# ChunLI-666/PointCloudProcessor

Hardware: AMD Instinct MI355X
Metric: Mpoints×frames/sec colorized (higher is better)
Workload: dtype f32/f64

## Files before the change

### include/pcp_hip.h

```cpp
#ifndef PCP_HIP_H
#define PCP_HIP_H

#include <stdint.h>

#ifdef __cplusplus
extern "C" {
#endif

#define PCP_ABI_VERSION 6

#define PCP_OK 0
#define PCP_ERR_INVALID (-1)
#define PCP_ERR_STATE (-2)
#define PCP_ERR_DEVICE (-3)
#define PCP_ERR_NOMEM (-4)
#define PCP_ERR_RANGE (-5)

typedef struct pcp_context pcp_context;

typedef struct pcp_pose {
  double x, y, z, qw, qx, qy, qz;
} pcp_pose;

typedef struct pcp_camera {
// ... 191 lines not shown
                   int64_t capacity, char *out_text, int64_t *out_bytes);
int pcp_colour_compact_ascii(pcp_context *ctx, int32_t with_label, int64_t first_row, int64_t max_rows, int64_t capacity,
                             char *out_text, int64_t *out_rows, int64_t *out_bytes);
int pcp_mls_fetch_ascii(pcp_context *ctx, int64_t first_row, int64_t max_rows, int64_t capacity, char *out_text,
                        int64_t *out_rows, int64_t *out_bytes);

#define PCP_ASCII_PARSE_MAX_ROW 65536
#define PCP_PARSE_LIMIT_ROW 0
#define PCP_PARSE_LIMIT_TILE 1
#define PCP_PARSE_LIMIT_PIECE 2
#define PCP_PARSE_LIMIT_TILE_ROWS 3
#define PCP_PARSE_LIMIT_WINDOW 4
int64_t pcp_ascii_parse_limit(int32_t which);
int pcp_ascii_parse_host(const char *text, int64_t bytes, int32_t columns, const int32_t col[4], int32_t final_window,
                         int64_t max_rows, float *out_x, float *out_y, float *out_z, float *out_intensity,
                         int64_t *out_rows, int64_t *out_consumed, int64_t *out_bad_row);
int pcp_ascii_parse(pcp_context *ctx, const char *text, int64_t bytes, int32_t columns, const int32_t col[4], int32_t final_window,
                    int64_t max_rows, float *out_x, float *out_y, float *out_z, float *out_intensity,
                    int64_t *out_rows, int64_t *out_consumed, int64_t *out_bad_row);

int pcp_close_pairs(pcp_context *ctx, double radius, int64_t *points_with_close_neighbour);

int pcp_timing_enable(pcp_context *ctx, int32_t on);
int pcp_timing_reset(pcp_context *ctx);
int pcp_timing_get(pcp_context *ctx, int32_t kernel_id, double *total_ms, int64_t *launches);
const char *pcp_kernel_name(int32_t kernel_id);
int pcp_tile_mask_density(pcp_context *ctx, double *kept_fraction);
int pcp_tile_masks(pcp_context *ctx, int64_t *tiles, int32_t *mask_words, uint32_t *out_words);
int pcp_sor_redo_fraction(pcp_context *ctx, double *fraction);
int pcp_sor_distances(pcp_context *ctx, int64_t capacity, float *out_distance);
int pcp_selftest_arithmetic(pcp_context *ctx, int64_t samples, uint64_t seed, int64_t *mismatches_fp64,
                            int64_t *mismatches_fp32);

#ifdef __cplusplus
}
#endif
#endif
```

### pointcloudprocessor_amd/capi.py

```python
from __future__ import annotations

import ctypes as C
import os
import re

import numpy as np

from . import _build

PCP_OK = 0
PCP_ERR_INVALID = -1
PCP_ERR_STATE = -2
PCP_ERR_DEVICE = -3
PCP_ERR_NOMEM = -4
PCP_ERR_RANGE = -5

NID_EVAL_FN = C.CFUNCTYPE(C.c_int, C.c_void_p, C.POINTER(C.c_double), C.c_int32, C.POINTER(C.c_double), C.POINTER(C.c_double),
                          C.POINTER(C.c_int32))
K_PROJECT, K_DEPTH, K_COLOUR, K_VISIBILITY, K_MLS_GRID, K_MLS_FIT, K_MISC, K_SOR, K_MLS_VOXEL, K_TILE_MASK, K_NID, K_HPR = range(12)
K_COLOUR_SMOOTH = 12
K_COUNT = 13


class PcpError(RuntimeError):
# ... 755 lines not shown
        Ti = np.ascontiguousarray(T_init, np.float64).reshape(16)
        out = np.zeros(16, np.float64)
        cost = C.c_double()
        evals = C.c_int32()
        rc = self.lib.pcp_nid_optimize_with(self.h, trampoline, None, _ptr(Ti), C.c_int32(bins), C.c_int32(max_outer_iterations),
                                            _ptr(out), C.byref(cost), C.byref(evals))
        if errors:
            raise errors[0]
        self._check(rc)
        return out.reshape(4, 4), cost.value, evals.value

    def timing_enable(self, on: bool = True):
        self._check(self.lib.pcp_timing_enable(self.h, C.c_int32(1 if on else 0)))

    def timing_reset(self):
        self._check(self.lib.pcp_timing_reset(self.h))

    def timing_get(self, kernel_id: int):
        ms = C.c_double()
        cnt = C.c_int64()
        self._check(self.lib.pcp_timing_get(self.h, C.c_int32(kernel_id), C.byref(ms), C.byref(cnt)))
        return ms.value, cnt.value

    def tile_mask_density(self) -> float:
        v = C.c_double()
        self._check(self.lib.pcp_tile_mask_density(self.h, C.byref(v)))
        return v.value

    def selftest_arithmetic(self, samples: int = 1 << 26, seed: int = 1):
        a, b = C.c_int64(), C.c_int64()
        self._check(self.lib.pcp_selftest_arithmetic(self.h, C.c_int64(samples), C.c_uint64(seed), C.byref(a), C.byref(b)))
        return a.value, b.value

    def tile_masks(self) -> np.ndarray:
        t, w = C.c_int64(), C.c_int32()
        self._check(self.lib.pcp_tile_masks(self.h, C.byref(t), C.byref(w), None))
        out = np.empty((t.value, w.value), np.uint32)
        self._check(self.lib.pcp_tile_masks(self.h, None, None, _ptr(out)))
        return out

    def kernel_name(self, kernel_id: int) -> str:
        return self.lib.pcp_kernel_name(C.c_int32(kernel_id)).decode()
```

### pointcloudprocessor_amd/csrc/pcp_colour.hip

```cpp
#include <algorithm>
#include <cfloat>
#include <cstdlib>

#include "pcp_device.hpp"
#include "pcp_hsv.hpp"
#include "pcp_scan.hpp"

namespace pcp {

constexpr int kBlock = 256;
constexpr uint32_t kFltMaxBits = 0x7f7fffffu;

template <bool kCommon>
__device__ __forceinline__ DevCamera common_camera(const DevCamera &in) {
  DevCamera c = in;
  if constexpr (kCommon) {
    c.cull_mode = PCP_CULL_ZBUFFER;
    c.enable_zbuf = 1;
    c.pretest = 1;
    c.ds_fast = 1;
  }
  return c;
}
inline bool is_common_camera(const DevCamera &c) {
// ... 291 lines not shown
  const uint32_t b = blockIdx.x;
  if (b >= (gridDim.x / kSuper) * kSuper) return b;
  const uint32_t x = b % kXcd, slot = b / kXcd;
  return ((slot / kXcdChunk) * kXcd + x) * kXcdChunk + slot % kXcdChunk;
}

constexpr unsigned long long kDepthEmpty = 0x7f7f7f7f7f7f7f7full;
__device__ __forceinline__ void depth_min(unsigned long long *__restrict__ map, int32_t cell, unsigned long long bits) {
  if (bits < map[cell]) atomicMin(map + cell, bits);
}
__device__ __forceinline__ double sumsq64(float xc, float yc, float zc) {
  const double X = xc, Y = yc, Z = zc;
  return (X * X + Y * Y) + Z * Z;
}
__global__ __launch_bounds__(kBlock) void k_depth_finish(const unsigned long long *__restrict__ sq, int64_t count,
                                                         uint32_t *__restrict__ range) {
  int64_t i = static_cast<int64_t>(blockIdx.x) * kBlock + threadIdx.x;
  const int64_t stride = static_cast<int64_t>(gridDim.x) * kBlock;
  for (; i < count; i += stride) {
    const unsigned long long b = sq[i];
    float r = FLT_MAX;
    if (b != kDepthEmpty) r = fminf(static_cast<float>(sqrt(__longlong_as_double(static_cast<long long>(b)))), FLT_MAX);
    range[i] = __float_as_uint(r);
  }
}

__device__ __forceinline__ uint32_t range_bits(int32_t w, int32_t f0, int32_t f1) {
  const int32_t fb = max(f0, w << 5), fe = min(f1, (w << 5) + 32);
  const int32_t nb = fe - fb;
  return nb <= 0 ? 0u : (((nb >= 32) ? 0xffffffffu : ((1u << nb) - 1u)) << (fb & 31));
}

template <bool kCommon>
__global__ __launch_bounds__(kBlock) void k_depth_pass(const float *__restrict__ x, const float *__restrict__ y,
                                                       const float *__restrict__ z, int64_t n, DevCamera cam_in,
                                                       const DevFrame *__restrict__ frames, int32_t f0, int32_t f1,
                                                       unsigned long long *__restrict__ depth, int64_t cells,
                                                       int32_t depth_first_frame, uint32_t *__restrict__ tile_mask,
                                                       const uint32_t *__restrict__ tile_inside, int32_t words,
                                                       const int32_t *__restrict__ tile_order) {
  DevCamera cam = common_camera<kCommon>(cam_in);
  if constexpr (kCommon) cam.pretest = 0;
  __shared__ unsigned long long combine[kBlock];
  const int lane = threadIdx.x & 63;
  unsigned long long *tbl = combine + (threadIdx.x & ~63);
  const int64_t j = tile_order ? static_cast<int64_t>(tile_order[blockIdx.x]) * 64 + threadIdx.x
                               : static_cast<int64_t>(xcd_chunked_block()) * kBlock + threadIdx.x;
  const bool live = j < n;
  if (!__ballot(live)) return;
  const float px = live ? x[j] : 0.0f, py = live ? y[j] : 0.0f, pz = live ? z[j] : 0.0f;
  const int64_t tile = __builtin_amdgcn_readfirstlane(static_cast<int32_t>(j >> 6));
  const bool finite_sure = cam.frames_bounded != 0 && __all(fabsf(px) <= 0x1p40f && fabsf(py) <= 0x1p40f && fabsf(pz) <= 0x1p40f);
  unsigned long long *held_at = nullptr;
  unsigned long long held_bits = 0ull, held_seen = 0ull;
  auto settle_held = [&]() {
    if (held_at && held_bits < held_seen) atomicMin(held_at, held_bits);
    held_at = nullptr;
  };
  for (int32_t w = f0 >> 5; w <= (f1 - 1) >> 5; ++w) {
    const uint32_t in_range = range_bits(w, f0, f1);
    uint32_t todo = in_range;
    if (tile_mask) todo &= tile_mask[tile * words + w];
    todo = __builtin_amdgcn_readfirstlane(todo);
    const uint32_t inside = tile_inside ? __builtin_amdgcn_readfirstlane(tile_inside[tile * words + w]) : 0u;
    uint32_t seen = 0u;
    while (todo) {
      const int32_t b = __builtin_ctz(todo);
      const int32_t f = (w << 5) + b;
      todo &= todo - 1u;
      const DevFrame &fr = frames[f];
      const Projected p = project_point(cam, fr.w2c, px, py, pz, ((inside >> b) & 1u) == 0u, finite_sure);
      const bool in_map = live && p.cell >= 0;
      const bool cand = live && p.pixel >= 0 && (cam.enable_zbuf ? p.cell >= 0 : p.cell != -1);
      if (__ballot(cand)) seen |= 1u << b;
      settle_held();
      if (cam.enable_zbuf && __ballot(in_map)) {
        unsigned long long *map = depth + static_cast<uint64_t>(static_cast<uint32_t>(f - depth_first_frame)) * static_cast<uint32_t>(cells);
        unsigned long long key = ~0ull, sbits = 0ull;
        if (in_map) {
          sbits = static_cast<unsigned long long>(__double_as_longlong(sumsq64(p.xc, p.yc, p.zc)));
          key = (static_cast<unsigned long long>(static_cast<uint32_t>(p.cell)) << 32) | (sbits >> 32);
        }
        tbl[lane] = ~0ull;
        __builtin_amdgcn_wave_barrier();
        if (in_map) atomicMin(&tbl[p.cell & 63], key);
        __builtin_amdgcn_wave_barrier();
        if (in_map) {
          const unsigned long long got = tbl[p.cell & 63];
          if (got == key || static_cast<uint32_t>(got >> 32) != static_cast<uint32_t>(p.cell)) {
            held_at = map + p.cell;
            held_bits = sbits;
            held_seen = *held_at;
          }
        }
        __builtin_amdgcn_wave_barrier();
      }
    }
    if (tile_mask && lane == 0 && live) {
      uint32_t *dst = tile_mask + tile * words + w;
      *dst = (*dst & ~in_range) | seen;
    }
  }
  settle_held();
}

__global__ __launch_bounds__(kBlock) void k_visibility(const float *__restrict__ x, const float *__restrict__ y,
                                                       const float *__restrict__ z, int64_t n, DevCamera cam,
                                                       DevFrame fr, const uint32_t *__restrict__ depth,
                                                       const int32_t *__restrict__ perm,
                                                       uint8_t *__restrict__ keep, int32_t require_pixel) {
  const int64_t i = static_cast<int64_t>(blockIdx.x) * kBlock + threadIdx.x;
  if (i >= n) return;
  const Projected p = project_point(cam, fr.w2c, x[i], y[i], z[i]);
  bool k = keep_rule(cam, p, depth);
  if (require_pixel) k = k && p.pixel >= 0;
  if (k) keep[perm ? perm[i] : i] = 1;
}

__device__ __forceinline__ bool keep_by_depth(float xc, float yc, float zc, double lim) {
  const double s = sumsq64(xc, yc, zc);
  const double L = lim * lim;
  bool keep = s < L * (1.0 - 0x1p-40);
  const bool sure = lim > 0.0 && (keep || s > L * (1.0 + 0x1p-40));
  if (!sure) keep = !(sqrt(s) > lim);
  return keep;
}

struct TopState {
  float *score;
  uint32_t *rgb;
  int32_t *frame;
  int32_t *count;
};

struct MatchArgs {
  const uint8_t *in_a;
  unsigned long long *moved;
  float e2;
// ... 224 lines not shown
  const uint64_t a = mix64(seed ^ static_cast<uint64_t>(i) * 3u), b = mix64(a);
  uint32_t bx = static_cast<uint32_t>(a), by = static_cast<uint32_t>(a >> 32), bz = static_cast<uint32_t>(b);
  const uint32_t mode = static_cast<uint32_t>(b >> 32) & 3u;
  if (mode != 0u) {
    const uint32_t span = mode == 1u ? 12u : 40u;
    bx = (bx & 0x807fffffu) | ((127u - span / 2u + (bx >> 23) % span) << 23);
    by = (by & 0x807fffffu) | ((127u - span / 2u + (by >> 23) % span) << 23);
    bz = (bz & 0x807fffffu) | ((127u - span / 2u + (bz >> 23) % span) << 23);
  }
  const float xc = __uint_as_float(bx), yc = __uint_as_float(by), zc = fabsf(__uint_as_float(bz));
  if (!(zc > 0.0f)) return;
  double xn, yn;
  divide_xy_by_z(xc, yc, zc, xn, yn);
  const double xr = static_cast<double>(xc) / static_cast<double>(zc);
  const double yr = static_cast<double>(yc) / static_cast<double>(zc);
  if (!same_f64(xn, xr) || !same_f64(yn, yr)) atomicAdd(bad, 1ull);
}

__global__ __launch_bounds__(kBlock) void k_selftest_div32(DevCamera cam, unsigned long long *__restrict__ bad) {
  const uint32_t lane = blockIdx.x * kBlock + threadIdx.x;
  uint32_t wrong = 0u;
  for (uint32_t k = 0; k < 256u; ++k) {
    const float x = __uint_as_float((k << 24) | lane);
    const float a = div_by_ds(cam, x), b = x / cam.ds_f;
    const float ax = fabsf(x);
    if (ax >= 0x1p-40f && ax <= 0x1p60f) {
      if (!((a != a && b != b) || __float_as_uint(a) == __float_as_uint(b))) ++wrong;
    } else {
      if (cell_of_quotient(a, cam.cull_wf) != cell_of_quotient(b, cam.cull_wf)) ++wrong;
      if (cell_of_quotient(a, cam.cull_hf) != cell_of_quotient(b, cam.cull_hf)) ++wrong;
    }
  }
  if (wrong) atomicAdd(bad, static_cast<unsigned long long>(wrong));
}

__global__ __launch_bounds__(kBlock) void k_unpack_result(const uint32_t *__restrict__ packed, int64_t n,
                                                         uint8_t *__restrict__ rgb, uint8_t *__restrict__ has) {
  const int64_t i = static_cast<int64_t>(blockIdx.x) * kBlock + threadIdx.x;
  if (i >= n) return;
  const uint32_t v = packed[i];
  rgb[3 * i + 0] = static_cast<uint8_t>(v & 0xffu);
  rgb[3 * i + 1] = static_cast<uint8_t>((v >> 8) & 0xffu);
  rgb[3 * i + 2] = static_cast<uint8_t>((v >> 16) & 0xffu);
  has[i] = static_cast<uint8_t>(v >> 24);
}

__global__ __launch_bounds__(kBlock) void k_unpack_labels(const uint32_t *__restrict__ packed, int64_t n,
                                                         uint8_t *__restrict__ label, uint8_t *__restrict__ hits,
                                                         uint8_t *__restrict__ views) {
  const int64_t i = static_cast<int64_t>(blockIdx.x) * kBlock + threadIdx.x;
  if (i >= n) return;
  const uint32_t v = packed[i];
  if (label) label[i] = static_cast<uint8_t>(v & 0xffu);
  if (hits) hits[i] = static_cast<uint8_t>((v >> 8) & 0xffu);
  if (views) views[i] = static_cast<uint8_t>((v >> 16) & 0xffu);
}

__global__ __launch_bounds__(kBlock) void k_fill_u32(uint32_t *__restrict__ p, int64_t n, uint32_t v) {
  int64_t i = static_cast<int64_t>(blockIdx.x) * kBlock + threadIdx.x;
  const int64_t stride = static_cast<int64_t>(gridDim.x) * kBlock;
  for (; i < n; i += stride) p[i] = v;
}

__global__ __launch_bounds__(kBlock) void k_scatter_u32(const uint32_t *__restrict__ in,
                                                        const int32_t *__restrict__ perm, int64_t n,
                                                        uint32_t *__restrict__ out) {
// ... 1322 lines not shown
}

int pcp_colour_labels_device(pcp_context *ctx, void **device_ptr, int64_t *n_words) {
  if (!ctx) return PCP_ERR_INVALID;
  if (!ctx->labels_live)
    return set_error(ctx, PCP_ERR_STATE, "pcp_colour_labels_device: no labels (pcp_set_label_fusion(1), then pcp_colorize / "
                     "pcp_colorize_from_depth / pcp_colour_finalise)");
  if (device_ptr) *device_ptr = ctx->labels.p;
  if (n_words) *n_words = ctx->n;
  return PCP_OK;
}

int pcp_selftest_arithmetic(pcp_context *ctx, int64_t samples, uint64_t seed, int64_t *mismatches_fp64,
                            int64_t *mismatches_fp32) {
  if (!ctx) return PCP_ERR_INVALID;
  if (!ctx->have_camera) return set_error(ctx, PCP_ERR_STATE, "pcp_selftest_arithmetic: pcp_set_camera has not been called");
  PCP_HIP_TRY(ctx, hipSetDevice(ctx->device));
  if (samples < 0) return set_error(ctx, PCP_ERR_INVALID, "pcp_selftest_arithmetic: negative sample count");
  PCP_HIP_TRY(ctx, ctx->s_counter.ensure(4));
  unsigned long long *bad = ctx->s_counter.p;
  PCP_HIP_TRY(ctx, hipMemsetAsync(bad, 0, 16, ctx->stream));
  if (samples > 0)
    hipLaunchKernelGGL(k_selftest_div64, dim3(blocks_for(samples)), dim3(kBlock), 0, ctx->stream, samples, seed, bad);
  hipLaunchKernelGGL(k_selftest_div32, dim3((1u << 24) / kBlock), dim3(kBlock), 0, ctx->stream, ctx->dcam, bad + 1);
  PCP_HIP_TRY(ctx, hipGetLastError());
  unsigned long long h[2] = {0, 0};
  PCP_HIP_TRY(ctx, hipMemcpyAsync(h, bad, 16, hipMemcpyDeviceToHost, ctx->stream));
  PCP_HIP_TRY(ctx, hipStreamSynchronize(ctx->stream));
  if (mismatches_fp64) *mismatches_fp64 = static_cast<int64_t>(h[0]);
  if (mismatches_fp32) *mismatches_fp32 = static_cast<int64_t>(h[1]);
  return PCP_OK;
}

}
```

### pointcloudprocessor_amd/csrc/pcp_context.hip

```cpp
#include <algorithm>
#include <cfloat>
#include <cmath>
#include <cstdlib>
#include <new>
#include <vector>

#include "pcp_internal.hpp"
#include "pcp_scan.hpp"

namespace pcp {

static thread_local std::string g_error;

int set_error(const pcp_context *ctx, int code, const char *fmt, ...) {
  char buf[1024];
  va_list ap;
  va_start(ap, fmt);
  vsnprintf(buf, sizeof(buf), fmt, ap);
  va_end(ap);
  if (ctx)
    ctx->error = buf;
  else
    g_error = buf;
  return code;
// ... 472 lines not shown
                       dx, dy, dz);
  } else if (aos) {
    PCP_HIP_TRY(ctx, raw.ensure(static_cast<size_t>(n) * static_cast<size_t>(stride) / 4 + 4));
    PCP_HIP_TRY(ctx, hipMemcpyAsync(raw.p, aos, static_cast<size_t>(n) * static_cast<size_t>(stride), hipMemcpyHostToDevice, st));
    hipLaunchKernelGGL(k_up_deinterleave, dim3(up_blocks(n)), dim3(kUpBlock), 0, st, raw.p, stride / 4, n, dx, dy, dz);
  } else {
    PCP_HIP_TRY(ctx, hipMemcpyAsync(dx, x, sn * 4, hipMemcpyHostToDevice, st));
    PCP_HIP_TRY(ctx, hipMemcpyAsync(dy, y, sn * 4, hipMemcpyHostToDevice, st));
    PCP_HIP_TRY(ctx, hipMemcpyAsync(dz, z, sn * 4, hipMemcpyHostToDevice, st));
  }
  float mn[3], mx[3];
  unsigned long long nonfinite = 0;
  PCP_HIP_TRY(ctx, ctx->inv_perm.ensure(plane + 4));
  if (int rc = spatial_order(ctx, dx, dy, dz, n, ctx->perm.p, ctx->sxyz.p, ctx->sxyz.p + plane, ctx->sxyz.p + 2 * plane,
                             ctx->inv_perm.p, mn, mx, &nonfinite))
    return rc;
  raw.release();
  ctx->nonfinite_points = static_cast<int64_t>(nonfinite);
  for (int a = 0; a < 3; ++a) {
    ctx->host_min[a] = mn[a];
    ctx->host_max[a] = mx[a];
  }
  const int64_t tiles = (n + 63) / 64, groups = (tiles + 15) / 16;
  PCP_HIP_TRY(ctx, ctx->tile_sphere.ensure(static_cast<size_t>(tiles + groups) * 4 + 4));
  float4 *sph = reinterpret_cast<float4 *>(ctx->tile_sphere.p);
  hipLaunchKernelGGL(k_up_spheres<64>, dim3(static_cast<uint32_t>((tiles + 3) / 4)), dim3(kUpBlock), 0, st, ctx->sxyz.p,
                     ctx->sxyz.p + plane, ctx->sxyz.p + 2 * plane, n, sph, tiles);
  hipLaunchKernelGGL(k_up_spheres<1024>, dim3(static_cast<uint32_t>(groups)), dim3(kUpBlock), 0, st, ctx->sxyz.p,
                     ctx->sxyz.p + plane, ctx->sxyz.p + 2 * plane, n, sph + tiles, groups);
  PCP_HIP_TRY(ctx, hipGetLastError());
  ctx->n_tiles = tiles;
  PCP_HIP_TRY(ctx, hipStreamSynchronize(st));
  return PCP_OK;
}

}

using namespace pcp;

extern "C" {

int pcp_abi_version(void) { return PCP_ABI_VERSION; }

int pcp_create(int32_t device, pcp_context **out) {
  if (!out) {
    set_global_error("pcp_create: out is NULL");
    return PCP_ERR_INVALID;
  }
  *out = nullptr;
  int count = 0;
  hipError_t e = hipGetDeviceCount(&count);
  if (e != hipSuccess || count <= 0) {
    set_global_error("pcp_create: no HIP device available (%s); libpcp_hip has no CPU fallback",
                     e == hipSuccess ? "device count 0" : hipGetErrorString(e));
    return PCP_ERR_DEVICE;
  }
  if (device < 0 || device >= count) {
    set_global_error("pcp_create: device %d out of range (0..%d)", device, count - 1);
    return PCP_ERR_INVALID;
  }
  e = hipSetDevice(device);
  if (e == hipSuccess) {
    hipFuncAttributes a;
    const hipError_t pl[] = {hipFuncGetAttributes(&a, reinterpret_cast<const void *>(&k_up_bbox)), preload_colour(), preload_mls(),
                             preload_nid(), preload_hpr(), preload_colour_smooth(), preload_match(),
                             preload_jpeg(), preload_stream_colour(), preload_ascii(), preload_ascii_parse()};
// ... 259 lines not shown
  d.cull_hf = static_cast<float>(cam->cull_height);
  d.mw = cam->cull_width / cp.downsample_factor;
  d.mh = cam->cull_height / cp.downsample_factor;
  d.cull_mode = cp.cull_mode == PCP_CULL_HPR ? PCP_CULL_HPR_CANDIDATES : cp.cull_mode;
  d.match_mode = cp.match_mode;
  d.cull_wd = static_cast<double>(cam->cull_width);
  d.cull_hd = static_cast<double>(cam->cull_height);
  {
    const double eps = static_cast<double>(1e-5f);
    d.match_r2 = static_cast<float>(eps * eps);
  }
  d.enable_zbuf = (cp.enable_depth_buffer_culling && cp.cull_mode == PCP_CULL_ZBUFFER) ? 1 : 0;
  d.pretest = 1;
  d.qfx = static_cast<float>(cam->fx);
  d.qfy = static_cast<float>(cam->fy);
  d.qcx = static_cast<float>(cam->cx);
  d.qcy = static_cast<float>(cam->cy);
  d.qk1 = static_cast<float>(cam->k1);
  d.qk2 = static_cast<float>(cam->k2);
  d.qk3 = static_cast<float>(cam->k3);
  d.qp1 = static_cast<float>(cam->p1);
  d.qp2 = static_cast<float>(cam->p2);
  {
    const float ds = static_cast<float>(cp.downsample_factor);
    const bool hpr = cp.cull_mode != PCP_CULL_ZBUFFER;
    const float cw = hpr ? static_cast<float>(d.cull_w) : ds * static_cast<float>(d.enable_zbuf ? d.mw : d.cull_w);
    const float ch = hpr ? static_cast<float>(d.cull_h) : ds * static_cast<float>(d.enable_zbuf ? d.mh : d.cull_h);
    d.u_lo = -(ds + 0.5f);
    d.v_lo = -(ds + 0.5f);
    d.u_hi = std::max(cw, static_cast<float>(d.img_w)) + 0.5f;
    d.v_hi = std::max(ch, static_cast<float>(d.img_h)) + 0.5f;
  }
  if (const char *e = std::getenv("PCP_DISABLE_PRETEST")) d.pretest = (e[0] == '1') ? 0 : 1;

  ctx->have_camera = true;
  for (hipStream_t us : ctx->upload_stream)
    if (us) (void)hipStreamSynchronize(us);
  std::fill(ctx->image_pending.begin(), ctx->image_pending.end(), uint8_t(0));
  ctx->image_set.assign(ctx->image_set.size(), 0);
  ctx->mask_set.assign(ctx->mask_set.size(), 0);
  std::fill(ctx->depth_valid.begin(), ctx->depth_valid.end(), uint8_t(0));
  ctx->hull_valid.clear();
  ctx->depth_accum.release();
  ctx->depth_accum_live = false;
  ctx->colour_state_live = false;
  ctx->colour_result_live = false;
  ctx->labels_live = false;
  return PCP_OK;
}

int pcp_upload_cloud(pcp_context *ctx, const float *x, const float *y, const float *z, int64_t n) {
  if (!ctx) return PCP_ERR_INVALID;
  if (n < 0 || n >= (int64_t(1) << 31)) return set_error(ctx, PCP_ERR_INVALID, "pcp_upload_cloud: n=%lld out of range", (long long)n);
  if (n > 0 && (!x || !y || !z)) return set_error(ctx, PCP_ERR_INVALID, "pcp_upload_cloud: NULL coordinate array");
  return store_cloud(ctx, x, y, z, n);
}

int pcp_upload_cloud_aos(pcp_context *ctx, const void *points, int64_t n, int64_t stride_bytes) {
  if (!ctx) return PCP_ERR_INVALID;
  if (n < 0 || n >= (int64_t(1) << 31)) return set_error(ctx, PCP_ERR_INVALID, "pcp_upload_cloud_aos: n out of range");
  if (stride_bytes < 12) return set_error(ctx, PCP_ERR_INVALID, "pcp_upload_cloud_aos: stride must be >= 12 bytes");
  if (n > 0 && !points) return set_error(ctx, PCP_ERR_INVALID, "pcp_upload_cloud_aos: NULL points");
  if (stride_bytes % 4 == 0 && (reinterpret_cast<uintptr_t>(points) & 3u) == 0)
    return store_cloud(ctx, nullptr, nullptr, nullptr, n, points, stride_bytes);
  std::vector<float> x(static_cast<size_t>(n)), y(static_cast<size_t>(n)), z(static_cast<size_t>(n));
  const uint8_t *base = static_cast<const uint8_t *>(points);
// ... 139 lines not shown
```

### pointcloudprocessor_amd/csrc/pcp_device.hpp

```cpp
#pragma once

#include <hip/hip_runtime.h>

#include <cfloat>
#include <cstdint>

#include "pcp_internal.hpp"

namespace pcp {

__device__ __forceinline__ void xform(const float *__restrict__ m, float x, float y, float z, float &xc, float &yc,
                                      float &zc) {
  xc = x * m[0] + (y * m[1] + (z * m[2] + m[3]));
  yc = x * m[4] + (y * m[5] + (z * m[6] + m[7]));
  zc = x * m[8] + (y * m[9] + (z * m[10] + m[11]));
}

__device__ __forceinline__ void divide_xy_by_z(float xc, float yc, float zc, double &xn, double &yn, bool finite_sure = false) {
  const double X = xc, Y = yc, Z = zc;
  if (finite_sure || (xc - xc) + (yc - yc) + (zc - zc) == 0.0f) {
    double r = __builtin_amdgcn_rcp(Z);
    double e = __builtin_fma(-Z, r, 1.0);
    r = __builtin_fma(r, e, r);
    e = __builtin_fma(-Z, r, 1.0);
// ... 62 lines not shown
  return ((cx < c.mw) & (cy < c.mh)) ? cy * c.mw + cx : (c.enable_zbuf ? -1 : -2);
}

__device__ __forceinline__ int32_t colour_pixel(const DevCamera &c, double u, double v) {
  if (!(u > -1.0 && u < c.img_wd && v > -1.0 && v < c.img_hd)) return -1;
  return static_cast<int32_t>(v) * c.img_w + static_cast<int32_t>(u);
}

__device__ __forceinline__ double range64(float xc, float yc, float zc) {
  const double X = xc, Y = yc, Z = zc;
  return sqrt((X * X + Y * Y) + Z * Z);
}

__device__ __forceinline__ bool surely_rejected(const DevCamera &c, float xc, float yc, float zc) {
  const float rz = __builtin_amdgcn_rcpf(zc);
  const float xn = xc * rz, yn = yc * rz;
  const float x2 = xn * xn, y2 = yn * yn;
  const float r2 = x2 + y2, r4 = r2 * r2, r6 = r2 * r4;
  const float rc = __builtin_fmaf(c.qk3, r6, __builtin_fmaf(c.qk2, r4, __builtin_fmaf(c.qk1, r2, 1.0f)));
  const float ra = __builtin_fmaf(fabsf(c.qk3), r6, __builtin_fmaf(fabsf(c.qk2), r4, __builtin_fmaf(fabsf(c.qk1), r2, 1.0f)));
  const float t1 = 2.0f * xn * yn;
  const float t2 = __builtin_fmaf(2.0f, x2, r2), t3 = __builtin_fmaf(2.0f, y2, r2);
  const float at1 = fabsf(t1);
  const float xd = __builtin_fmaf(c.qp2, t2, __builtin_fmaf(c.qp1, t1, rc * xn));
  const float yd = __builtin_fmaf(c.qp2, t1, __builtin_fmaf(c.qp1, t3, rc * yn));
  const float sx = __builtin_fmaf(fabsf(c.qp2), t2, __builtin_fmaf(fabsf(c.qp1), at1, ra * fabsf(xn)));
  const float sy = __builtin_fmaf(fabsf(c.qp2), at1, __builtin_fmaf(fabsf(c.qp1), t3, ra * fabsf(yn)));
  const float u = __builtin_fmaf(c.qfx, xd, c.qcx), v = __builtin_fmaf(c.qfy, yd, c.qcy);
  constexpr float kErr = 1.52587890625e-05f;
  const float eu = kErr * __builtin_fmaf(fabsf(c.qfx), sx, fabsf(c.qcx));
  const float ev = kErr * __builtin_fmaf(fabsf(c.qfy), sy, fabsf(c.qcy));
  const float over = fmaxf(fmaxf(c.u_lo - (u + eu), (u - eu) - c.u_hi), fmaxf(c.v_lo - (v + ev), (v - ev) - c.v_hi));
  return over > 0.0f;
}

struct Projected {
  float xc, yc, zc;
  int32_t cell;
  int32_t pixel;
};

template <bool kPretest = true, bool kShortDiv = true>
__device__ __forceinline__ Projected project_point(const DevCamera &c, const float *__restrict__ m, float x, float y,
                                                   float z, bool pretest_here = true, bool finite_sure = false) {
  Projected p;
  xform(m, x, y, z, p.xc, p.yc, p.zc);
  p.cell = -1;
  p.pixel = -1;
  if (p.zc > 0.0f && !(kPretest && pretest_here && c.pretest && surely_rejected(c, p.xc, p.yc, p.zc))) {
    double u, v;
    project_uv<kShortDiv>(c, p.xc, p.yc, p.zc, u, v, finite_sure);
    p.cell = cull_cell<kShortDiv>(c, u, v);
    p.pixel = colour_pixel(c, u, v);
  }
  return p;
}

__device__ __forceinline__ bool keep_rule(const DevCamera &c, const Projected &p, const uint32_t *__restrict__ depth) {
  if (!c.enable_zbuf) return p.cell != -1;
  if (p.cell < 0) return false;
  const double r = range64(p.xc, p.yc, p.zc);
  const double lim = static_cast<double>(__uint_as_float(depth[p.cell])) + c.slack;
  return !(r > lim);
}

__device__ __forceinline__ bool roundtrip_sample(const DevCamera &c, const DevFrame &fr, float wx0, float wy0, float wz0,
// ... 149 lines not shown
```

### pointcloudprocessor_amd/csrc/pcp_internal.hpp

```cpp
#pragma once

#include <hip/hip_runtime.h>

#include <cstdarg>
#include <cstdint>
#include <chrono>
#include <cstdio>
#include <cstring>
#include <string>
#include <vector>

#include "pcp_hip.h"

namespace pcp {

struct DevCamera {
  double fx, fy, cx, cy;
  double k1, k2, p1, p2, k3;
  double slack;
  float ds_f;
  double img_wd, img_hd;
  float cull_wf, cull_hf;
  float ds_rcp;
  int32_t ds_fast;
  int32_t ds;
  int32_t img_w, img_h;
  int32_t cull_w, cull_h;
  int32_t mw, mh;
  int32_t enable_zbuf;
  int32_t cull_mode;
  int32_t match_mode;
  double cull_wd, cull_hd;
  float match_r2;
  int32_t pretest;
  int32_t frames_bounded;
  float qfx, qfy, qcx, qcy;
  float qk1, qk2, qk3, qp1, qp2;
  float u_lo, u_hi, v_lo, v_hi;
};

struct DevFrame {
  float w2c[12];
  float c2w[12];
  double px, py, pz;
  double norm_bound;
  float c2w_inv[12];
  float pad_[4];
};
static_assert(sizeof(DevFrame) == 192, "DevFrame layout");

constexpr int kTopM = 5;

struct TimingSlot {
  double total_ms = 0.0;
  int64_t launches = 0;
};

struct PendingEvent {
  hipEvent_t start, stop;
  int32_t kernel;
};

struct AllocTally {
  double seconds = 0.0, bytes = 0.0;
};
inline AllocTally &alloc_tally() {
  static AllocTally t;
  return t;
}
struct AllocClock {
  std::chrono::steady_clock::time_point t0 = std::chrono::steady_clock::now();
// ... 341 lines not shown
```

Measured before the change: 1.860 million.

## Add fp32 fast cell classification with deferred exact projection in depth pass

Adds a host-computed error-bounded fp32 classifier that decides a point's depth cell, or that it is outside the map, without the fp64 projection. Points it cannot decide are queued per wavefront in a shared-memory ring and reprojected exactly in batches of 64 via lane permutes. The common-camera depth pass also claims tile-mask words atomically and pins the SGPR budget. This aims to cut fp64 divide and projection work per point-frame, at the cost of more complexity, ring bookkeeping and a selftest entry point to validate the classifier's bounds.

```diff
diff --git a/include/pcp_hip.h b/include/pcp_hip.h
--- a/include/pcp_hip.h
+++ b/include/pcp_hip.h
@@ -247,6 +247,9 @@
 int pcp_selftest_arithmetic(pcp_context *ctx, int64_t samples, uint64_t seed, int64_t *mismatches_fp64,
                             int64_t *mismatches_fp32);
 
+int pcp_selftest_cells(pcp_context *ctx, const float *xc, const float *yc, const float *zc, int64_t given, int64_t samples,
+                       uint64_t seed, int64_t counts[5]);
+
 #ifdef __cplusplus
 }
 #endif
diff --git a/pointcloudprocessor_amd/capi.py b/pointcloudprocessor_amd/capi.py
--- a/pointcloudprocessor_amd/capi.py
+++ b/pointcloudprocessor_amd/capi.py
@@ -811,6 +811,18 @@
         self._check(self.lib.pcp_selftest_arithmetic(self.h, C.c_int64(samples), C.c_uint64(seed), C.byref(a), C.byref(b)))
         return a.value, b.value
 
+    def selftest_cells(self, points=None, samples: int = 1 << 20, seed: int = 1):
+        x = y = z = None
+        n = 0
+        if points is not None and len(points):
+            pts = np.asarray(points, np.float32)
+            x, y, z = (np.ascontiguousarray(pts[:, k]) for k in range(3))
+            n = len(x)
+        out = (C.c_int64 * 5)()
+        self._check(self.lib.pcp_selftest_cells(self.h, _ptr(x), _ptr(y), _ptr(z), C.c_int64(n), C.c_int64(samples),
+                                                C.c_uint64(seed), out))
+        return dict(zip(("mismatches", "unsure", "tested", "in_map", "in_map_unsure"), (int(v) for v in out)))
+
     def tile_masks(self) -> np.ndarray:
         t, w = C.c_int64(), C.c_int32()
         self._check(self.lib.pcp_tile_masks(self.h, C.byref(t), C.byref(w), None))
diff --git a/pointcloudprocessor_amd/csrc/pcp_colour.hip b/pointcloudprocessor_amd/csrc/pcp_colour.hip
--- a/pointcloudprocessor_amd/csrc/pcp_colour.hip
+++ b/pointcloudprocessor_amd/csrc/pcp_colour.hip
@@ -347,13 +347,13 @@
 }
 
 template <bool kCommon>
-__global__ __launch_bounds__(kBlock) void k_depth_pass(const float *__restrict__ x, const float *__restrict__ y,
-                                                       const float *__restrict__ z, int64_t n, DevCamera cam_in,
-                                                       const DevFrame *__restrict__ frames, int32_t f0, int32_t f1,
-                                                       unsigned long long *__restrict__ depth, int64_t cells,
-                                                       int32_t depth_first_frame, uint32_t *__restrict__ tile_mask,
-                                                       const uint32_t *__restrict__ tile_inside, int32_t words,
-                                                       const int32_t *__restrict__ tile_order) {
+__device__ __forceinline__ void depth_pass_body(const float *__restrict__ x, const float *__restrict__ y,
+                                                const float *__restrict__ z, int64_t n, const DevCamera &cam_in,
+                                                const DevFrame *__restrict__ frames, int32_t f0, int32_t f1,
+                                                unsigned long long *__restrict__ depth, int64_t cells,
+                                                int32_t depth_first_frame, uint32_t *__restrict__ tile_mask,
+                                                const uint32_t *__restrict__ tile_inside, int32_t words,
+                                                const int32_t *__restrict__ tile_order) {
   DevCamera cam = common_camera<kCommon>(cam_in);
   if constexpr (kCommon) cam.pretest = 0;
   __shared__ unsigned long long combine[kBlock];
@@ -372,6 +372,98 @@
     if (held_at && held_bits < held_seen) atomicMin(held_at, held_bits);
     held_at = nullptr;
   };
+  if constexpr (kCommon) {
+    if (cam.fc_on && finite_sure) {
+      __shared__ uint32_t unsure_ring[kBlock / 64][128];
+      uint32_t *ring = unsure_ring[threadIdx.x >> 6];
+      uint32_t head = 0u, waiting = 0u;
+      uint32_t *tile_words = tile_mask ? tile_mask + tile * words : nullptr;
+      auto drain = [&](uint32_t count) {
+        settle_held();
+        __builtin_amdgcn_wave_barrier();
+        const bool mine = static_cast<uint32_t>(lane) < count;
+        const uint32_t entry = mine ? ring[(head + static_cast<uint32_t>(lane)) & 127u] : static_cast<uint32_t>(lane);
+        const int32_t owner4 = static_cast<int32_t>(entry & 63u) << 2;
+        const float ox = __int_as_float(__builtin_amdgcn_ds_bpermute(owner4, __float_as_int(px)));
+        const float oy = __int_as_float(__builtin_amdgcn_ds_bpermute(owner4, __float_as_int(py)));
+        const float oz = __int_as_float(__builtin_amdgcn_ds_bpermute(owner4, __float_as_int(pz)));
+        if (mine) {
+          const int32_t f = static_cast<int32_t>(entry >> 6);
+          float m[12];
+#pragma unroll
+          for (int k = 0; k < 12; ++k) m[k] = frames[f].w2c[k];
+          const Projected p = project_point<false>(cam, m, ox, oy, oz, false, true);
+          if (p.cell >= 0) {
+            depth_min(depth + static_cast<uint64_t>(static_cast<uint32_t>(f - depth_first_frame)) * static_cast<uint32_t>(cells), p.cell,
+                      static_cast<unsigned long long>(__double_as_longlong(sumsq64(p.xc, p.yc, p.zc))));
+            if (tile_words && p.pixel >= 0) atomicOr(tile_words + (f >> 5), 1u << (f & 31));
+          }
+        }
+        head = (head + count) & 127u;
+        waiting -= count;
+      };
+      for (int32_t w = f0 >> 5; w <= (f1 - 1) >> 5; ++w) {
+        const uint32_t in_range = range_bits(w, f0, f1);
+        uint32_t todo = in_range;
+        if (tile_words) {
+          uint32_t was = 0u;
+          if (lane == 0) was = atomicAnd(tile_words + w, ~in_range);
+          todo &= __builtin_amdgcn_readfirstlane(was);
+        }
+        uint32_t seen = 0u;
+        while (todo) {
+          const int32_t b = __builtin_ctz(todo);
+          const int32_t f = (w << 5) + b;
+          todo &= todo - 1u;
+          const DevFrame &fr = frames[f];
+          float xc, yc, zc;
+          xform(fr.w2c, px, py, pz, xc, yc, zc);
+          const bool front = live && zc > 0.0f;
+          int32_t cell;
+          bool cand;
+          const bool sure = classify_cell(cam, xc, yc, zc, cell, cand);
+          const bool unsure = front && !sure;
+          const bool in_map = front && sure && cell >= 0;
+          if (__ballot(in_map && cand)) seen |= 1u << b;
+          const unsigned long long um = __ballot(unsure);
+          if (um) {
+            if (unsure) {
+              const uint32_t at = __builtin_amdgcn_mbcnt_hi(static_cast<uint32_t>(um >> 32), __builtin_amdgcn_mbcnt_lo(static_cast<uint32_t>(um), 0u));
+              ring[(head + waiting + at) & 127u] = (static_cast<uint32_t>(f) << 6) | static_cast<uint32_t>(lane);
+            }
+            waiting += static_cast<uint32_t>(__popcll(um));
+          }
+          settle_held();
+          if (__ballot(in_map)) {
+            unsigned long long *map = depth + static_cast<uint64_t>(static_cast<uint32_t>(f - depth_first_frame)) * static_cast<uint32_t>(cells);
+            unsigned long long key = ~0ull, sbits = 0ull;
+            if (in_map) {
+              sbits = static_cast<unsigned long long>(__double_as_longlong(sumsq64(xc, yc, zc)));
+              key = (static_cast<unsigned long long>(static_cast<uint32_t>(cell)) << 32) | (sbits >> 32);
+            }
+            tbl[lane] = ~0ull;
+            __builtin_amdgcn_wave_barrier();
+            if (in_map) atomicMin(&tbl[cell & 63], key);
+            __builtin_amdgcn_wave_barrier();
+            if (in_map) {
+              const unsigned long long got = tbl[cell & 63];
+              if (got == key || static_cast<uint32_t>(got >> 32) != static_cast<uint32_t>(cell)) {
+                held_at = map + cell;
+                held_bits = sbits;
+                held_seen = *held_at;
+              }
+            }
+            __builtin_amdgcn_wave_barrier();
+          }
+          if (waiting >= 64u) drain(64u);
+        }
+        if (tile_words && seen && lane == 0) atomicOr(tile_words + w, seen);
+      }
+      if (waiting) drain(waiting);
+      settle_held();
+      return;
+    }
+  }
   for (int32_t w = f0 >> 5; w <= (f1 - 1) >> 5; ++w) {
     const uint32_t in_range = range_bits(w, f0, f1);
     uint32_t todo = in_range;
@@ -419,6 +511,27 @@
   settle_held();
 }
 
+template <bool kCommon>
+__global__ __launch_bounds__(kBlock) void k_depth_pass(const float *__restrict__ x, const float *__restrict__ y,
+                                                       const float *__restrict__ z, int64_t n, DevCamera cam_in,
+                                                       const DevFrame *__restrict__ frames, int32_t f0, int32_t f1,
+                                                       unsigned long long *__restrict__ depth, int64_t cells,
+                                                       int32_t depth_first_frame, uint32_t *__restrict__ tile_mask,
+                                                       const uint32_t *__restrict__ tile_inside, int32_t words,
+                                                       const int32_t *__restrict__ tile_order) {
+  depth_pass_body<kCommon>(x, y, z, n, cam_in, frames, f0, f1, depth, cells, depth_first_frame, tile_mask, tile_inside, words,
+                           tile_order);
+}
+template <>
+__global__ __launch_bounds__(kBlock) __attribute__((amdgpu_num_sgpr(102))) void k_depth_pass<true>(
+    const float *__restrict__ x, const float *__restrict__ y, const float *__restrict__ z, int64_t n, DevCamera cam_in,
+    const DevFrame *__restrict__ frames, int32_t f0, int32_t f1, unsigned long long *__restrict__ depth, int64_t cells,
+    int32_t depth_first_frame, uint32_t *__restrict__ tile_mask, const uint32_t *__restrict__ tile_inside, int32_t words,
+    const int32_t *__restrict__ tile_order) {
+  depth_pass_body<true>(x, y, z, n, cam_in, frames, f0, f1, depth, cells, depth_first_frame, tile_mask, tile_inside, words,
+                        tile_order);
+}
+
 __global__ __launch_bounds__(kBlock) void k_visibility(const float *__restrict__ x, const float *__restrict__ y,
                                                        const float *__restrict__ z, int64_t n, DevCamera cam,
                                                        DevFrame fr, const uint32_t *__restrict__ depth,
@@ -709,6 +822,79 @@
     }
   }
   if (wrong) atomicAdd(bad, static_cast<unsigned long long>(wrong));
+}
+
+__device__ __forceinline__ double selftest_hug(const DevCamera &cam, uint64_t r, int32_t img, int32_t cells) {
+  const double ds = cam.ds_f;
+  const uint32_t kind = static_cast<uint32_t>(r & 15u);
+  const double unit = static_cast<double>((r >> 8) & 0xffffffu) * 0x1p-24;
+  const double off = (((r >> 4) & 1u) ? 1.0 : -1.0) * exp2(-3.0 - 20.0 * static_cast<double>((r >> 32) & 0xffffu) * 0x1p-16) ;
+  switch (kind) {
+    case 0: return -1.0 + off;
+    case 1: return 0.0 + off;
+    case 2: return img - 1.0 + off;
+    case 3: return img + off;
+    case 4: return -ds + off;
+    case 5: return ds * cells + off;
+    case 6: return -ds * unit;
+    case 7: case 8: return (img + 2.0 * ds) * unit - ds;
+    default: return ds * static_cast<double>((r >> 40) % static_cast<uint32_t>(cells + 1)) + off;
+  }
+}
+__global__ __launch_bounds__(kBlock) void k_selftest_cells(DevCamera cam_in, const float *__restrict__ gx, const float *__restrict__ gy,
+                                                           const float *__restrict__ gz, int64_t given, int64_t total, uint64_t seed,
+                                                           unsigned long long *__restrict__ out) {
+  const DevCamera cam = common_camera<true>(cam_in);
+  const int64_t i = static_cast<int64_t>(blockIdx.x) * kBlock + threadIdx.x;
+  float xc = 0.0f, yc = 0.0f, zc = -1.0f;
+  if (i < given) {
+    xc = gx[i];
+    yc = gy[i];
+    zc = gz[i];
+  } else if (i < total) {
+    const uint64_t a = mix64(seed ^ static_cast<uint64_t>(i) * 3u), b = mix64(a), c = mix64(b);
+    const double depth = exp2(-2.0 + 7.0 * static_cast<double>(c >> 40) * 0x1p-24);
+    double xn, yn;
+    if (a % 3u == 0u) {
+      xn = (static_cast<double>(b >> 40) * 0x1p-23 - 1.0) * 2.0 * cam.fc_xmax;
+      yn = (static_cast<double>((b >> 16) & 0xffffffu) * 0x1p-23 - 1.0) * 2.0 * cam.fc_ymax;
+    } else {
+      const double xt = (selftest_hug(cam, b, cam.img_w, cam.mw) - cam.cx) / cam.fx;
+      const double yt = (selftest_hug(cam, c, cam.img_h, cam.mh) - cam.cy) / cam.fy;
+      xn = xt;
+      yn = yt;
+      for (int it = 0; it < 12; ++it) {
+        const double x2 = xn * xn, y2 = yn * yn, r2 = x2 + y2;
+        const double rc = 1.0 + r2 * (cam.k1 + r2 * (cam.k2 + r2 * cam.k3));
+        const double t1 = 2.0 * xn * yn;
+        xn = (xt - cam.p1 * t1 - cam.p2 * (r2 + 2.0 * x2)) / rc;
+        yn = (yt - cam.p1 * (r2 + 2.0 * y2) - cam.p2 * t1) / rc;
+      }
+    }
+    zc = static_cast<float>(depth);
+    xc = static_cast<float>(xn * static_cast<double>(zc));
+    yc = static_cast<float>(yn * static_cast<double>(zc));
+  }
+  const bool tested = zc > 0.0f && (xc - xc) + (yc - yc) + (zc - zc) == 0.0f;
+  bool wrong = false, unsure = false, in_map = false;
+  if (tested) {
+    int32_t cell = -1;
+    bool cand = false;
+    const bool sure = cam.fc_on != 0 && classify_cell(cam, xc, yc, zc, cell, cand);
+    double u, v;
+    project_uv(cam, xc, yc, zc, u, v);
+    const int32_t ecell = cull_cell(cam, u, v);
+    const bool ecand = ecell >= 0 && colour_pixel(cam, u, v) >= 0;
+    in_map = ecell >= 0;
+    unsure = !sure;
+    wrong = sure && (cell != ecell || cand != ecand);
+  }
+  const bool flags[5] = {wrong, unsure, tested, in_map, in_map && unsure};
+#pragma unroll
+  for (int k = 0; k < 5; ++k) {
+    const unsigned long long m = __ballot(flags[k]);
+    if (m && (threadIdx.x & 63) == 0) atomicAdd(out + k, static_cast<unsigned long long>(__popcll(m)));
+  }
 }
 
 __global__ __launch_bounds__(kBlock) void k_unpack_result(const uint32_t *__restrict__ packed, int64_t n,
@@ -2097,4 +2283,37 @@
   return PCP_OK;
 }
 
-}
+int pcp_selftest_cells(pcp_context *ctx, const float *xc, const float *yc, const float *zc, int64_t given, int64_t samples,
+                       uint64_t seed, int64_t *counts) {
+  if (!ctx) return PCP_ERR_INVALID;
+  if (!ctx->have_camera) return set_error(ctx, PCP_ERR_STATE, "pcp_selftest_cells: pcp_set_camera has not been called");
+  if (given < 0 || samples < 0 || given + samples >= (int64_t(1) << 31) || !counts || (given > 0 && (!xc || !yc || !zc)))
+    return set_error(ctx, PCP_ERR_INVALID, "pcp_selftest_cells: bad arguments");
+  if (ctx->dcam.cull_mode != PCP_CULL_ZBUFFER || !ctx->dcam.enable_zbuf || !ctx->dcam.ds_fast)
+    return set_error(ctx, PCP_ERR_STATE, "pcp_selftest_cells: the classification belongs to the z-buffer cull with its depth buffer and "
+                     "the short divisions on");
+  PCP_HIP_TRY(ctx, hipSetDevice(ctx->device));
+  PCP_HIP_TRY(ctx, ctx->s_counter.ensure(8));
+  PCP_HIP_TRY(ctx, ctx->s_cam.ensure(static_cast<size_t>(std::max<int64_t>(given, 1)) * 3));
+  unsigned long long *out = ctx->s_counter.p;
+  PCP_HIP_TRY(ctx, hipMemsetAsync(out, 0, 40, ctx->stream));
+  float *g = ctx->s_cam.p;
+  if (given > 0) {
+    const size_t bytes = static_cast<size_t>(given) * 4;
+    PCP_HIP_TRY(ctx, hipMemcpyAsync(g, xc, bytes, hipMemcpyHostToDevice, ctx->stream));
+    PCP_HIP_TRY(ctx, hipMemcpyAsync(g + given, yc, bytes, hipMemcpyHostToDevice, ctx->stream));
+    PCP_HIP_TRY(ctx, hipMemcpyAsync(g + 2 * given, zc, bytes, hipMemcpyHostToDevice, ctx->stream));
+  }
+  const int64_t total = given + samples;
+  if (total > 0)
+    hipLaunchKernelGGL(k_selftest_cells, dim3(blocks_for(total)), dim3(kBlock), 0, ctx->stream, ctx->dcam, g, g + given, g + 2 * given,
+                       given, total, seed, out);
+  PCP_HIP_TRY(ctx, hipGetLastError());
+  unsigned long long h[5] = {0, 0, 0, 0, 0};
+  PCP_HIP_TRY(ctx, hipMemcpyAsync(h, out, 40, hipMemcpyDeviceToHost, ctx->stream));
+  PCP_HIP_TRY(ctx, hipStreamSynchronize(ctx->stream));
+  for (int k = 0; k < 5; ++k) counts[k] = static_cast<int64_t>(h[k]);
+  return PCP_OK;
+}
+
+}
diff --git a/pointcloudprocessor_amd/csrc/pcp_context.hip b/pointcloudprocessor_amd/csrc/pcp_context.hip
--- a/pointcloudprocessor_amd/csrc/pcp_context.hip
+++ b/pointcloudprocessor_amd/csrc/pcp_context.hip
@@ -528,6 +528,54 @@
   ctx->n_tiles = tiles;
   PCP_HIP_TRY(ctx, hipStreamSynchronize(st));
   return PCP_OK;
+}
+
+static float f32_up(double v) {
+  float f = static_cast<float>(v);
+  return static_cast<double>(f) < v ? std::nextafterf(f, INFINITY) : f;
+}
+static float f32_down(double v) {
+  float f = static_cast<float>(v);
+  return static_cast<double>(f) > v ? std::nextafterf(f, -INFINITY) : f;
+}
+static void set_fast_cells(DevCamera &d) {
+  d.fc_on = 0;
+  d.fc_xmax = d.fc_ymax = 0.0f;
+  d.fc_d = 1.0f;
+  d.fc_omd = 0.0f;
+  d.fc_out_lo = -INFINITY;
+  d.fc_out_hi_u = d.fc_out_hi_v = INFINITY;
+  const float q[9] = {d.qfx, d.qfy, d.qcx, d.qcy, d.qk1, d.qk2, d.qk3, d.qp1, d.qp2};
+  for (float v : q)
+    if (!std::isfinite(v)) return;
+  if (!d.ds_fast || d.ds < 1 || d.mw < 1 || d.mh < 1 || d.qfx == 0.0f || d.qfy == 0.0f) return;
+  const double ds = d.ds_f;
+  const double fx = std::fabs(d.qfx), fy = std::fabs(d.qfy), cx = std::fabs(d.qcx), cy = std::fabs(d.qcy);
+  const double k1 = std::fabs(d.qk1), k2 = std::fabs(d.qk2), k3 = std::fabs(d.qk3), p1 = std::fabs(d.qp1), p2 = std::fabs(d.qp2);
+  auto half_span = [&](double hi, double c, double f) { return std::min(1.5 * std::max(std::fabs(-ds - c), std::fabs(hi - c)) / f, 64.0); };
+  d.fc_xmax = f32_down(half_span(ds * (d.mw + 1), d.qcx, fx));
+  d.fc_ymax = f32_down(half_span(ds * (d.mh + 1), d.qcy, fy));
+  const double X = d.fc_xmax, Y = d.fc_ymax;
+  const double x2 = X * X, y2 = Y * Y, r2 = x2 + y2, r4 = r2 * r2, r6 = r2 * r4;
+  const double ra = 1.0 + k1 * r2 + k2 * r4 + k3 * r6;
+  const double t1 = 2.0 * X * Y, t2 = r2 + 2.0 * x2, t3 = r2 + 2.0 * y2;
+  const double sx = ra * X + p1 * t1 + p2 * t2, sy = ra * Y + p1 * t3 + p2 * t1;
+  const double su = fx * sx + cx, sv = fy * sy + cy;
+  const double widen = 1.0 + 0x1p-16;
+  const double eu = 0x1p-16 * su * widen, ev = 0x1p-16 * sv * widen;
+  for (double v : {ra, sx, sy, su, sv, r6, k3 * r6, p1 * t3, p2 * t2})
+    if (!(v < 0x1p100)) return;
+  if (!(eu < 0.5 && ev < 0.5 && eu > 0x1p-60 && ev > 0x1p-60)) return;
+  const double slop = (std::max(d.mw, d.mh) + 2) * 0x1p-21;
+  const double dd = (std::max(eu, ev) / ds + slop) * widen;
+  if (!(dd < 0.25)) return;
+  if (static_cast<int64_t>(d.ds) * d.mw > d.img_w || static_cast<int64_t>(d.ds) * d.mh > d.img_h) return;
+  d.fc_out_lo = f32_down(-1.0 - dd);
+  d.fc_out_hi_u = f32_up(d.mw + dd);
+  d.fc_out_hi_v = f32_up(d.mh + dd);
+  d.fc_d = f32_up(std::max(dd, std::max(static_cast<double>(d.fc_out_hi_u) - d.mw, static_cast<double>(d.fc_out_hi_v) - d.mh)));
+  d.fc_omd = f32_down(1.0 - static_cast<double>(d.fc_d));
+  d.fc_on = 1;
 }
 
 }
@@ -853,6 +901,7 @@
     d.v_hi = std::max(ch, static_cast<float>(d.img_h)) + 0.5f;
   }
   if (const char *e = std::getenv("PCP_DISABLE_PRETEST")) d.pretest = (e[0] == '1') ? 0 : 1;
+  set_fast_cells(d);
 
   ctx->have_camera = true;
   for (hipStream_t us : ctx->upload_stream)
diff --git a/pointcloudprocessor_amd/csrc/pcp_device.hpp b/pointcloudprocessor_amd/csrc/pcp_device.hpp
--- a/pointcloudprocessor_amd/csrc/pcp_device.hpp
+++ b/pointcloudprocessor_amd/csrc/pcp_device.hpp
@@ -118,6 +118,31 @@
   const float ev = kErr * __builtin_fmaf(fabsf(c.qfy), sy, fabsf(c.qcy));
   const float over = fmaxf(fmaxf(c.u_lo - (u + eu), (u - eu) - c.u_hi), fmaxf(c.v_lo - (v + ev), (v - ev) - c.v_hi));
   return over > 0.0f;
+}
+
+__device__ __forceinline__ bool classify_cell(const DevCamera &c, float xc, float yc, float zc, int32_t &cell, bool &cand) {
+  const float rz = __builtin_amdgcn_rcpf(zc);
+  const float xn = xc * rz, yn = yc * rz;
+  const float axn = fabsf(xn), ayn = fabsf(yn);
+  const bool boxed = (axn <= c.fc_xmax) & (ayn <= c.fc_ymax);
+  const float x2 = xn * xn, y2 = yn * yn;
+  const float r2 = x2 + y2, r4 = r2 * r2, r6 = r2 * r4;
+  const float rc = __builtin_fmaf(c.qk3, r6, __builtin_fmaf(c.qk2, r4, __builtin_fmaf(c.qk1, r2, 1.0f)));
+  const float t1 = 2.0f * xn * yn;
+  const float t2 = __builtin_fmaf(2.0f, x2, r2), t3 = __builtin_fmaf(2.0f, y2, r2);
+  const float xd = __builtin_fmaf(c.qp2, t2, __builtin_fmaf(c.qp1, t1, rc * xn));
+  const float yd = __builtin_fmaf(c.qp2, t1, __builtin_fmaf(c.qp1, t3, rc * yn));
+  const float u = __builtin_fmaf(c.qfx, xd, c.qcx), v = __builtin_fmaf(c.qfy, yd, c.qcy);
+  const float qu = u * c.ds_rcp, qv = v * c.ds_rcp;
+  const float ku = __builtin_floorf(qu), kv = __builtin_floorf(qv);
+  const float fu = qu - ku, fv = qv - kv;
+  const float over = fmaxf(fmaxf(c.fc_out_lo - qu, qu - c.fc_out_hi_u), fmaxf(c.fc_out_lo - qv, qv - c.fc_out_hi_v));
+  const bool within = !(over > 0.0f);
+  const bool outside = !within;
+  const bool inside = (fu > c.fc_d) & (fu < c.fc_omd) & (fv > c.fc_d) & (fv < c.fc_omd) & (qu > c.fc_d) & (qv > c.fc_d) & within;
+  cand = inside;
+  cell = inside ? static_cast<int32_t>(kv) * c.mw + static_cast<int32_t>(ku) : -1;
+  return boxed & (inside | outside);
 }
 
 struct Projected {
diff --git a/pointcloudprocessor_amd/csrc/pcp_internal.hpp b/pointcloudprocessor_amd/csrc/pcp_internal.hpp
--- a/pointcloudprocessor_amd/csrc/pcp_internal.hpp
+++ b/pointcloudprocessor_amd/csrc/pcp_internal.hpp
@@ -37,6 +37,11 @@
   float qfx, qfy, qcx, qcy;
   float qk1, qk2, qk3, qp1, qp2;
   float u_lo, u_hi, v_lo, v_hi;
+  int32_t fc_on;
+  float fc_xmax, fc_ymax;
+  float fc_d, fc_omd;
+  float fc_out_lo;
+  float fc_out_hi_u, fc_out_hi_v;
 };
 
 struct DevFrame {
```

Measured after the change: 1.821 million. 0.979x the previous value.
